# naver/panst3r

Measured on AMD Instinct MI355X. Metric: frames/sec (whole node), N-view 512px panoptic inference, higher is better.
Workload: dtype f16

## Files before the change

### include/panst3r_hip.h

```cpp
#ifndef PANST3R_HIP_H
#define PANST3R_HIP_H
#include <stdint.h>
#ifdef __cplusplus
extern "C" {
#endif

#define PST_ABI_VERSION 20

#define PST_BF16 0
#define PST_F32  1
#define PST_F16  2
#define PST_X3H  4

int pst_abi_version(void);
const char* pst_last_error(void);

typedef struct pst_gemm_params {
  const void* A;  int64_t lda;
  const void* W;  int64_t ldw;
  void* C;        int64_t ldc;
  int32_t M, N, K;
  const float* bias;
  const float* gamma;
  const float* res;  int64_t ldr;
// ... 6 lines not shown
  int32_t conv_c, conv_h, conv_w;
  const void* zeros;
  const int32_t* rope_pos; const float* rope_cs; int32_t rope_hd;
  int32_t rope_npos;
  int32_t res_bf16;
  int32_t kernel;
  int32_t batch;
  int64_t a_bs, w_bs, c_bs, bias_bs;
  int32_t dtype16;
  void* xcopy; int64_t ldxc;
  float* stats_out; int32_t stats_ld;
  const float* ln_stats; int32_t ln_groups; const float* ln_colsum; float ln_eps;
  int32_t x3_block;
} pst_gemm_params;

int pst_gemm(const pst_gemm_params* p, void* stream);
const char* pst_gemm_variant(const pst_gemm_params* p);
int pst_gemm_pair(const pst_gemm_params* a, const pst_gemm_params* b, void* stream);
const char* pst_gemm_pair_variant(const pst_gemm_params* a, const pst_gemm_params* b);
#define PST_TUNE_G256_PP 3
#define PST_TUNE_PAIR 4
#define PST_TUNE_DEEP_RING 8
#define PST_TUNE_PAIR_ATTN 7
#define PST_TUNE_ATTN_XCD 9
#define PST_TUNE_CUS 10
#define PST_TUNE_PAIR_DELAY 6
#define PST_TUNE_DEPHASE 11
#define PST_TUNE_PAIR_RES 5
int pst_tune(int knob, int value);

int pst_mask_head_supported(int Q, int P, int C);
int pst_mask_head(const void* E, int64_t lde, const void* F, int64_t f_view_stride, float* out, int64_t out_view_stride, int nviews, int Q, int P, int C,
                  int dtype16, void* stream);

typedef struct pst_attn_params {
  const void* Q;  int64_t q_bs, q_hs, q_rs;
  const void* K;  int64_t k_bs, k_hs, k_rs;
  const void* Vt; int64_t v_bs, v_hs, v_ds;
  void* O;        int64_t o_bs, o_hs, o_rs;
  const uint8_t* mask; int64_t m_bs, m_rs;
  int32_t B, H, Nq, Nk, hd;
  float scale;
  const void* zeros;
  int32_t nsplit;
  void* ws; int64_t ws_bytes;
  int32_t dtype16;
  int32_t prescaled;
} pst_attn_params;

int64_t pst_attn_workspace_bytes(int B, int H, int Nq, int hd, int nsplit);

int pst_attn_fwd(const pst_attn_params* p, void* stream);
const char* pst_attn_variant(const pst_attn_params* p);
int pst_attn_pair(const pst_attn_params* a, const pst_attn_params* b, void* stream);
const char* pst_attn_pair_variant(const pst_attn_params* a, const pst_attn_params* b);

int pst_layernorm(const void* x, int64_t ldx, int in_fp32, void* y, int64_t ldy, int out_fp32,
                  const float* gamma, const float* beta, int rows, int D, float eps,
                  int grp_in, int grp_out, int grp_off, void* stream);
int pst_layernorm_add(const void* x, int64_t ldx, int in_fp32, const float* add, int64_t ld_add, void* y, int64_t ldy,
                      int out_fp32, const float* gamma, const float* beta, int rows, int D, float eps,
                      int grp_in, int grp_out, int grp_off, void* stream);

int pst_token_embed(const int32_t* ids, int B, int L, const float* tok, int vocab, const float* pos, int npos, int D, float* out, int64_t ldo,
                    int32_t* status, void* stream);

int pst_rowstats(const void* x, int64_t ldx, int x_type, void* xcopy, int64_t ldxc, float* stats, int stats_ld, int rows, int D, int dtype16,
                 void* stream);

int pst_layernorm_add_batch(const void* x, int64_t ldx, int in_fp32, const float* add, int64_t ld_add, void* y, int64_t ldy,
                            int out_fp32, const float* gamma, const float* beta, int rows, int D, float eps,
                            int grp_in, int grp_out, int grp_off, int nbatch, int64_t x_bs, int64_t y_bs, int64_t w_bs,
                            void* stream);

int pst_split3(const float* x, int64_t ldx, void* out, int64_t ldo, int rows, int K, int dtype16, void* stream);

int pst_split_operand(const float* x, int64_t ldx, void* out, int64_t ldo, int rows, int K, int Kpad, int side, int dtype16, void* stream);
int pst_split2(const float* x, int64_t ldx, void* hi, void* lo, int64_t ldo, int rows, int K, int transpose, int dtype16, void* stream);
int pst_transpose_f32(const float* x, int64_t ldx, float* y, int64_t ldy, int rows, int cols, void* stream);
int pst_rope2d_split(const float* x, int64_t ld, const int32_t* pos, const float* cs, void* hi, void* lo, int64_t ldo, int rows, int nheads, int hd, int dtype16,
                     void* stream);
int pst_attn_x3(const pst_attn_params* p, const void* Q_lo, const void* K_lo, const void* Vt_lo, int out_type, int64_t out_block, void* stream);
const char* pst_attn_x3_variant(const pst_attn_params* p);

int pst_rope2d(void* x, int64_t ld, const int32_t* pos, const float* cs, int rows, int nheads, int hd, int dtype16,
               void* stream);

int pst_patchify(const float* img, void* out, int64_t ld, int nimg, int C, int H, int W, int p, int dtype16, void* stream);
int pst_dino_preprocess(const float* img, float* out, int nimg, int H, int W, int Ho, int Wo, void* stream);

int pst_image_prepare(const uint8_t* src, int Hs, int Ws, float* dst, int Hr, int Wr, int top, int left, int H, int W, void* stream);
int pst_patch_rows(const float* img, void* enc, int64_t ld_enc, void* dino, int64_t ld_dino, int nimg, int H, int W, int p_enc, int p_dino,
                   int dino_transposed, int dtype16, void* stream);

int pst_add_cast(const void* a, int64_t lda, int a_fp32, const void* b, int64_t ldb, int b_fp32, int b_mod,
                 void* y, int64_t ldy, int y_fp32, int rows, int D, void* stream);
int pst_l2norm_rows(const float* x, int64_t ldx, void* y, int64_t ldy, int rows, int D, float eps, int dtype16, void* stream);

int pst_mean4(const void* F, void* Fm, int nimg, int Hm, int Wm, int C, int dtype16, void* stream);
int pst_resize_bilinear(const void* F, void* Fd, int nimg, int Hs, int Ws, int Hd, int Wd, int C, int dtype16, void* stream);
int pst_attn_mask_from_logits(const float* logits, int64_t ldl, uint8_t* mask, int64_t ldm, int Q, int Nk,
                              void* stream);

#define PST_STATS_BLOCKS 128
int pst_loftup_guidance_gn(const float* img, const float* biases, const float* gamma, const float* beta, float eps,
                           float* scratch, float* stats, void* y, int64_t ldy, int nimg, int H, int W, int nf, int dtype16,
// ... 215 lines not shown
```

### panst3r_amd/csrc/attention.hip

```cpp
#include "common.h"
#include "../../include/panst3r_hip.h"

namespace pst {

constexpr int KT = 64;
constexpr float NEG = -1e30f;

template <int HD>
struct AttnCfg {
  static constexpr int KPITCH = (HD == 64) ? 128 : 256;
  static constexpr int KSLOTS = KPITCH / 16;
  static constexpr int KCHUNKS = HD / 8;
  static constexpr int K_BYTES = KT * KPITCH;
  static constexpr int V_BYTES = HD * 128;
  static constexpr int BUF = K_BYTES + V_BYTES;
  __device__ static __forceinline__ int kswz(int row) { return (HD == 64) ? ((row >> 1) & 7) : (row & 15); }
};

__device__ __forceinline__ float max_rows(float v) {
  const unsigned u = __float_as_uint(v);
  const auto a = __builtin_amdgcn_permlane16_swap(u, u, false, false);
  float m;
  asm("v_max_f32 %0, %1, %2" : "=v"(m) : "v"(a[0]), "v"(a[1]));
  const unsigned w = __float_as_uint(m);
  const auto b = __builtin_amdgcn_permlane32_swap(w, w, false, false);
  asm("v_max_f32 %0, %1, %2" : "=v"(m) : "v"(b[0]), "v"(b[1]));
  return m;
}

template <int HD, int QF, bool F16, bool PRE>
__device__ __forceinline__ void attn_body(const pst_attn_params& p, const int bidx, char* smem) {
  using C = AttnCfg<HD>;
  constexpr int NKK = HD / 32;
  constexpr int NHF = HD / 16;

  const int tid = threadIdx.x, lane = tid & 63;
  const int wave = __builtin_amdgcn_readfirstlane(tid >> 6);
  const int g = lane >> 4, l16 = lane & 15;

  const int qblocks = (p.Nq + 64 * QF - 1) / (64 * QF);
  const int nsplit = p.nsplit > 1 ? p.nsplit : 1;
  const int split = bidx % nsplit;
  const int bid = bidx / nsplit;
  const int qb = bid % qblocks, bh = bid / qblocks;
  const int h = bh % p.H, b = bh / p.H;

  const bf16_t* Qp = (const bf16_t*)p.Q + (int64_t)b * p.q_bs + (int64_t)h * p.q_hs;
  const bf16_t* Kp = (const bf16_t*)p.K + (int64_t)b * p.k_bs + (int64_t)h * p.k_hs;
  const bf16_t* Vp = (const bf16_t*)p.Vt + (int64_t)b * p.v_bs + (int64_t)h * p.v_hs;
  bf16_t* Op = (bf16_t*)p.O + (int64_t)b * p.o_bs + (int64_t)h * p.o_hs;
  const uint8_t* Mp = p.mask ? p.mask + (int64_t)b * p.m_bs : nullptr;

  const int q_wave0 = qb * (64 * QF) + wave * (16 * QF);
  bf16x8 qf[QF][NKK];
#pragma unroll
  for (int a = 0; a < QF; ++a) {
    const int q = min(q_wave0 + a * 16 + l16, p.Nq - 1);
#pragma unroll
    for (int kk = 0; kk < NKK; ++kk) qf[a][kk] = *(const bf16x8*)(Qp + (int64_t)q * p.q_rs + kk * 32 + g * 8);
  }

  constexpr int K_PER_THR = KT * C::KSLOTS / 256;
  constexpr int V_PER_THR = HD * 8 / 256;
  int k_key[K_PER_THR], k_chunk[K_PER_THR];
#pragma unroll
  for (int j = 0; j < K_PER_THR; ++j) {
    const int c = j * 256 + tid, row = c / C::KSLOTS, pos = c % C::KSLOTS;
    const int f = row >> 4, i = row & 15;
    k_key[j] = (f >> 1) * 32 + (i >> 2) * 8 + (f & 1) * 4 + (i & 3);
    k_chunk[j] = pos ^ C::kswz(row);
  }
  int v_row[V_PER_THR], v_chunk[V_PER_THR];
#pragma unroll
  for (int j = 0; j < V_PER_THR; ++j) {
    const int c = j * 256 + tid, row = c >> 3, pos = c & 7;
    v_row[j] = row;
    v_chunk[j] = pos ^ ((row >> 1) & 7);
  }

  uint32_t k_off[K_PER_THR], v_off[V_PER_THR];
#pragma unroll
  for (int j = 0; j < K_PER_THR; ++j) k_off[j] = (uint32_t)(k_key[j] * (int)p.k_rs + k_chunk[j] * 8) * 2u;
#pragma unroll
  for (int j = 0; j < V_PER_THR; ++j) v_off[j] = (uint32_t)(v_row[j] * (int)p.v_ds + v_chunk[j] * 8) * 2u;
  auto stage = [&](int kt, int buf) {
    const int k0 = kt * KT;
    char* kd = smem + buf * C::BUF + wave * 1024;
    char* vd = smem + buf * C::BUF + C::K_BYTES + wave * 1024;
    if (k0 + KT <= p.Nk) {
      const char* kbase = (const char*)Kp + (int64_t)k0 * p.k_rs * 2;
      const char* vbase = (const char*)Vp + (int64_t)k0 * 2;
#pragma unroll
      for (int j = 0; j < K_PER_THR; ++j)
        if (C::KSLOTS == C::KCHUNKS || k_chunk[j] < C::KCHUNKS) glds16(kbase + k_off[j], kd + j * 4096);
#pragma unroll
      for (int j = 0; j < V_PER_THR; ++j) glds16(vbase + v_off[j], vd + j * 4096);
      return;
    }
#pragma unroll
    for (int j = 0; j < K_PER_THR; ++j) {
      if (C::KSLOTS == C::KCHUNKS || k_chunk[j] < C::KCHUNKS) {
        const int key = min(k0 + k_key[j], p.Nk - 1);
        glds16(Kp + (int64_t)key * p.k_rs + k_chunk[j] * 8, kd + j * 4096);
      }
    }
#pragma unroll
    for (int j = 0; j < V_PER_THR; ++j) {
      const int kcol = k0 + v_chunk[j] * 8;
      const bf16_t* s = (kcol < p.Nk) ? Vp + (int64_t)v_row[j] * p.v_ds + kcol : (const bf16_t*)p.zeros;
      glds16(s, vd + j * 4096);
    }
  };

  f32x4 o[NHF][QF];
#pragma unroll
  for (int hf = 0; hf < NHF; ++hf)
#pragma unroll
    for (int a = 0; a < QF; ++a) o[hf][a] = f32x4{0.f, 0.f, 0.f, 0.f};
  f32x4 negm[QF];
  float m_run[QF], lsum[QF];
  float sum_lim[QF];
#pragma unroll
  for (int a = 0; a < QF; ++a) { m_run[a] = NEG; negm[a] = f32x4{0.f, 0.f, 0.f, 0.f}; lsum[a] = 0.f; sum_lim[a] = -1.0f; }
  bf16x8 ones;
  {
    union { bf16x8 v; uint32_t u[4]; } t;
    t.u[0] = t.u[1] = t.u[2] = t.u[3] = F16 ? 0x3c003c00u : 0x3f803f80u;
    ones = t.v;
    asm volatile("" : "+v"(ones));
  }

  const float c_exp = PRE ? 1.0f : p.scale * 1.4426950408889634f;
  const float lazy_thr = 8.0f / c_exp;
  const int tiles_all = (p.Nk + KT - 1) / KT;
  const int tps = (tiles_all + nsplit - 1) / nsplit;
  const int kt_begin = split * tps;
  const int ntiles = min(tiles_all, kt_begin + tps);
  if (kt_begin < ntiles) stage(kt_begin, 0);
  for (int kt = kt_begin; kt < ntiles; ++kt) {
#ifndef PST_ABL_NOSTAGE
    wait_vm0();
    __syncthreads();
    if (kt + 1 < ntiles) stage(kt + 1, (kt + 1 - kt_begin) & 1);
    const char* kb_ = smem + ((kt - kt_begin) & 1) * C::BUF;
#else
    if (kt == kt_begin) { wait_vm0(); __syncthreads(); }
    const char* kb_ = smem;
#endif
    const char* vb_ = kb_ + C::K_BYTES;
    const int k0 = kt * KT;
    if (q_wave0 >= p.Nq) continue;

    const bool tail = (k0 + KT > p.Nk);
    bool fast = !Mp && !tail && kt > kt_begin;
    bool trip[QF];
#pragma unroll
    for (int a = 0; a < QF; ++a) trip[a] = false;
    bf16x8 pb[QF][2];
    f32x4 tsum[QF];
    for (;;) {
      asm volatile("" ::: "memory");
      f32x4 s[4][QF];
#pragma unroll
      for (int f = 0; f < 4; ++f) {
#pragma unroll
        for (int a = 0; a < QF; ++a) s[f][a] = negm[a];
        const int row = f * 16 + l16;
#pragma unroll
        for (int kk = 0; kk < NKK; ++kk) {
          const int kc = kk * 4 + g;
          const bf16x8 kf = *(const bf16x8*)(kb_ + row * C::KPITCH + ((kc ^ C::kswz(row)) << 4));
#pragma unroll
          for (int a = 0; a < QF; ++a) s[f][a] = H16<F16>::mfma(kf, qf[a][kk], s[f][a]);
        }
      }

      if (!fast) {
        int k0c = k0;
        asm volatile("" : "+s"(k0c));
        float mx[QF];
#pragma unroll
        for (int a = 0; a < QF; ++a) {
          const int q = q_wave0 + a * 16 + l16;
          if (Mp || tail) {
            const uint8_t* mrow = Mp ? Mp + (int64_t)min(q, p.Nq - 1) * p.m_rs : nullptr;
#pragma unroll
            for (int f = 0; f < 4; ++f) {
              const int key = k0c + (f >> 1) * 32 + g * 8 + (f & 1) * 4;
              uint32_t mb = 0;
              if (mrow && key < p.Nk) mb = *(const uint32_t*)(mrow + key);
#pragma unroll
              for (int r = 0; r < 4; ++r)
                if (key + r >= p.Nk || ((mb >> (8 * r)) & 0xff)) s[f][a][r] = NEG;
            }
          }
          auto max3 = [](float x, float y, float z) { return fmaxf(fmaxf(x, y), z); };
          float m0 = max3(s[0][a][0], s[0][a][1], s[0][a][2]), m1 = max3(s[2][a][0], s[2][a][1], s[2][a][2]);
          m0 = max3(m0, s[0][a][3], s[1][a][0]); m1 = max3(m1, s[2][a][3], s[3][a][0]);
          m0 = max3(m0, s[1][a][1], s[1][a][2]); m1 = max3(m1, s[3][a][1], s[3][a][2]);
          mx[a] = fmaxf(max3(m0, m1, s[1][a][3]), s[3][a][3]);
        }
// ... 28 lines not shown
      }

#pragma unroll
      for (int a = 0; a < QF; ++a) {
        float pv[4][4];
#pragma unroll
        for (int f = 0; f < 4; ++f)
#pragma unroll
          for (int r = 0; r < 4; ++r) {
#ifndef PST_ABL_NOEXP
            pv[f][r] = __builtin_amdgcn_exp2f(PRE ? s[f][a][r] : s[f][a][r] * c_exp);
#else
            pv[f][r] = s[f][a][r];
#endif
          }
#pragma unroll
        for (int kb = 0; kb < 2; ++kb) {
          union { bf16x8 v; uint32_t u[4]; } pk;
          pk.u[0] = H16<F16>::pack(pv[2 * kb][0], pv[2 * kb][1]);
          pk.u[1] = H16<F16>::pack(pv[2 * kb][2], pv[2 * kb][3]);
          pk.u[2] = H16<F16>::pack(pv[2 * kb + 1][0], pv[2 * kb + 1][1]);
          pk.u[3] = H16<F16>::pack(pv[2 * kb + 1][2], pv[2 * kb + 1][3]);
          pb[a][kb] = pk.v;
        }
        tsum[a] = H16<F16>::mfma(ones, pb[a][0], f32x4{0.f, 0.f, 0.f, 0.f});
        tsum[a] = H16<F16>::mfma(ones, pb[a][1], tsum[a]);
      }
      if (!fast) break;
      uint64_t tripped = 0;
#pragma unroll
      for (int a = 0; a < QF; ++a) {
        trip[a] = !(tsum[a][0] <= sum_lim[a]);
        tripped |= __builtin_amdgcn_ballot_w64(trip[a]);
      }
      if (tripped == 0) break;
      fast = false;
    }

#pragma unroll
    for (int a = 0; a < QF; ++a) lsum[a] += tsum[a][0];
#pragma unroll
    for (int hf = 0; hf < NHF; ++hf) {
      const int row = hf * 16 + l16;
#pragma unroll
      for (int kb = 0; kb < 2; ++kb) {
        const int vc = kb * 4 + g;
        const bf16x8 vf = *(const bf16x8*)(vb_ + row * 128 + ((vc ^ ((row >> 1) & 7)) << 4));
#pragma unroll
        for (int a = 0; a < QF; ++a) o[hf][a] = H16<F16>::mfma(vf, pb[a][kb], o[hf][a]);
      }
    }
  }

  if (nsplit > 1) {
    float* ws_o = (float*)p.ws;
    const int64_t rows = (int64_t)p.B * p.H * p.Nq;
    float* ws_ml = ws_o + (int64_t)nsplit * rows * HD;
#pragma unroll
    for (int a = 0; a < QF; ++a) {
      const float l = lsum[a];
      const int q = q_wave0 + a * 16 + l16;
      if (q < p.Nq) {
        const int64_t row = ((int64_t)b * p.H + h) * p.Nq + q;
        float* dst = ws_o + ((int64_t)split * rows + row) * HD + 4 * g;
#pragma unroll
        for (int hf = 0; hf < NHF; ++hf) *(float4*)(dst + hf * 16) = make_float4(o[hf][a][0], o[hf][a][1], o[hf][a][2], o[hf][a][3]);
        if (g == 0) *(float2*)(ws_ml + ((int64_t)split * rows + row) * 2) = make_float2(m_run[a], l);
      }
    }
    return;
  }

#pragma unroll
  for (int a = 0; a < QF; ++a) {
    const float l = lsum[a];
    const float inv = l > 0.f ? 1.0f / l : 0.f;
    const int q = q_wave0 + a * 16 + l16;
    if (q < p.Nq) {
      bf16_t* dst = Op + (int64_t)q * p.o_rs + 4 * g;
#pragma unroll
      for (int hf = 0; hf < NHF; ++hf)
        *(uint2*)(dst + hf * 16) = make_uint2(H16<F16>::pack(o[hf][a][0] * inv, o[hf][a][1] * inv),
                                              H16<F16>::pack(o[hf][a][2] * inv, o[hf][a][3] * inv));
    }
  }
}

template <int HD, int QF, bool F16, bool PRE>
__global__ __launch_bounds__(256) void attn_kernel(const pst_attn_params p, const int xcd) {
  extern __shared__ __attribute__((aligned(16))) char smem[];
  attn_body<HD, QF, F16, PRE>(p, xcd ? xcd_remap((int)blockIdx.x, (int)gridDim.x) : (int)blockIdx.x, smem);
}

struct attn2_args {
  pst_attn_params p[2];
  int nblk0;
};
template <int HD, int QF, bool F16, bool PRE>
__global__ __launch_bounds__(256) void attn2_kernel(const attn2_args a, const int xcd) {
  extern __shared__ __attribute__((aligned(16))) char smem[];
  const int blk = xcd ? xcd_remap((int)blockIdx.x, (int)gridDim.x) : (int)blockIdx.x;
  const int which = blk >= a.nblk0 ? 1 : 0;
  attn_body<HD, QF, F16, PRE>(a.p[which], which ? blk - a.nblk0 : blk, smem);
}

__global__ void attn_combine_kernel(const pst_attn_params p, int hd) {
  const int64_t rows = (int64_t)p.B * p.H * p.Nq;
  const int per_row = hd / 4;
  const int64_t total = rows * per_row;
  const float c_exp = p.prescaled ? 1.0f : p.scale * 1.4426950408889634f;
  const float* ws_o = (const float*)p.ws;
  const float* ws_ml = ws_o + (int64_t)p.nsplit * rows * hd;
  for (int64_t i = blockIdx.x * (int64_t)blockDim.x + threadIdx.x; i < total; i += (int64_t)gridDim.x * blockDim.x) {
    const int64_t row = i / per_row;
    const int d = (int)(i - row * per_row) * 4;
    float m = NEG;
    for (int s = 0; s < p.nsplit; ++s) m = fmaxf(m, ws_ml[((int64_t)s * rows + row) * 2]);
    float l = 0.f, acc[4] = {0.f, 0.f, 0.f, 0.f};
    for (int s = 0; s < p.nsplit; ++s) {
      const float2 ml = *(const float2*)(ws_ml + ((int64_t)s * rows + row) * 2);
      const float wgt = __builtin_amdgcn_exp2f((ml.x - m) * c_exp);
      const float4 v = *(const float4*)(ws_o + ((int64_t)s * rows + row) * hd + d);
      l += ml.y * wgt;
      acc[0] += v.x * wgt; acc[1] += v.y * wgt; acc[2] += v.z * wgt; acc[3] += v.w * wgt;
    }
    const float inv = l > 0.f ? 1.0f / l : 0.f;
    const int q = (int)(row % p.Nq);
    const int bh = (int)(row / p.Nq), h = bh % p.H, b = bh / p.H;
    bf16_t* dst = (bf16_t*)p.O + (int64_t)b * p.o_bs + (int64_t)h * p.o_hs + (int64_t)q * p.o_rs + d;
    *(uint2*)dst = make_uint2(pack2(acc[0] * inv, acc[1] * inv, p.dtype16), pack2(acc[2] * inv, acc[3] * inv, p.dtype16));
  }
}

static int g_attn_xcd = 1;
int attn_xcd_order(int set) { const int prev = g_attn_xcd; if (set == 0 || set == 1) g_attn_xcd = set; return prev; }

template <int HD, int QF, bool F16, bool PRE>
static int launch_attn4(const pst_attn_params& p, hipStream_t s) {
  const int qblocks = (p.Nq + 64 * QF - 1) / (64 * QF);
  const int nsplit = p.nsplit > 1 ? p.nsplit : 1;
  const long grid = (long)qblocks * p.H * p.B * nsplit;
  hipLaunchKernelGGL((attn_kernel<HD, QF, F16, PRE>), dim3((unsigned)grid), dim3(256), 2 * AttnCfg<HD>::BUF, s, p, attn_xcd_order(-1));
  if (nsplit > 1) {
    const int64_t total = (int64_t)p.B * p.H * p.Nq * (HD / 4);
    int64_t g = (total + 255) / 256;
    if (g > 4096) g = 4096;
    hipLaunchKernelGGL(attn_combine_kernel, dim3((unsigned)g), dim3(256), 0, s, p, HD);
  }
  return check_launch("attn_fwd");
}

template <int HD, int QF, bool F16>
static int launch_attn(const pst_attn_params& p, hipStream_t s) {
  return p.prescaled ? launch_attn4<HD, QF, F16, true>(p, s) : launch_attn4<HD, QF, F16, false>(p, s);
}

template <int HD, int QF, bool F16, bool PRE>
static int launch_attn2_t(const pst_attn_params& pa, const pst_attn_params& pb, hipStream_t s) {
  attn2_args a;
  a.p[0] = pa; a.p[1] = pb;
  const long ga = (long)((pa.Nq + 64 * QF - 1) / (64 * QF)) * pa.H * pa.B, gb = (long)((pb.Nq + 64 * QF - 1) / (64 * QF)) * pb.H * pb.B;
  a.nblk0 = (int)ga;
  hipLaunchKernelGGL((attn2_kernel<HD, QF, F16, PRE>), dim3((unsigned)(ga + gb)), dim3(256), 2 * AttnCfg<HD>::BUF, s, a, attn_xcd_order(-1));
  return check_launch("attn_fwd (pair)");
}

int attn_f32_validate(const pst_attn_params& p);
int launch_attn_f32(const pst_attn_params& p, hipStream_t s);

}

static int attn_validate(const pst_attn_params* pp) {
  using namespace pst;
  if (!pp) { set_error("attn: null params"); return PST_EINVAL; }
  const pst_attn_params& p = *pp;
  if (p.dtype16 == DT_F32) {
    if (p.prescaled != 0 && p.prescaled != 1) { set_error("attn: prescaled must be 0 or 1"); return PST_EINVAL; }
    if (!p.prescaled && !(p.scale > 0.f)) { set_error("attn: scale must be positive"); return PST_EINVAL; }
    if (p.B <= 0 || p.H <= 0 || p.Nq <= 0 || p.Nk <= 0 || !p.Q || !p.K || !p.Vt || !p.O) { set_error("attn: bad shape / null operand"); return PST_EINVAL; }
    return attn_f32_validate(p);
  }
  if (p.dtype16 != DT_BF16 && p.dtype16 != DT_F16) { set_error("attn: dtype16 must be PST_BF16, PST_F16 or PST_F32"); return PST_EINVAL; }
  if (p.prescaled != 0 && p.prescaled != 1) { set_error("attn: prescaled must be 0 or 1"); return PST_EINVAL; }
  if (!p.prescaled && !(p.scale > 0.f)) { set_error("attn: scale must be positive"); return PST_EINVAL; }
  if (p.hd != 64 && p.hd != 96) { set_error("attn: head dim %d unsupported (64 or 96)", p.hd); return PST_EINVAL; }
  if (p.B <= 0 || p.H <= 0 || p.Nq <= 0 || p.Nk <= 0) { set_error("attn: bad shape"); return PST_EINVAL; }
  if (!p.Q || !p.K || !p.Vt || !p.O || !p.zeros) { set_error("attn: null operand"); return PST_EINVAL; }
  if ((p.q_rs | p.q_hs | p.q_bs | p.k_rs | p.k_hs | p.k_bs | p.v_ds | p.v_hs | p.v_bs) % 8) {
    set_error("attn: Q/K/Vt strides must be multiples of 8 elements (16-byte rows)"); return PST_EINVAL;
  }
  if ((p.o_rs | p.o_hs | p.o_bs) % 4) { set_error("attn: O strides must be multiples of 4"); return PST_EINVAL; }
  if (((uintptr_t)p.Q | (uintptr_t)p.K | (uintptr_t)p.Vt) & 15 || ((uintptr_t)p.O & 7)) {
    set_error("attn: operands must be 16-byte aligned"); return PST_EINVAL;
  }
  if (p.k_rs < 0) { set_error("attn: k_rs must not be negative"); return PST_EINVAL; }
  if (p.v_ds < 0) { set_error("attn: v_ds must not be negative"); return PST_EINVAL; }
  if (p.k_rs * 64 * 2 >= (1ll << 31) || p.v_ds * (int64_t)p.hd * 2 >= (1ll << 31)) { set_error("attn: K row / V^T row stride too large"); return PST_EINVAL; }
  if (p.mask && ((p.m_rs | p.m_bs) % 4 || ((uintptr_t)p.mask & 3))) { set_error("attn: mask rows must be 4-byte aligned"); return PST_EINVAL; }
  if (p.nsplit > 1) {
    const int64_t need = (int64_t)p.nsplit * p.B * p.H * p.Nq * (p.hd + 2) * 4;
    if (!p.ws || p.ws_bytes < need || ((uintptr_t)p.ws & 15)) { set_error("attn: split-K needs a 16-byte aligned workspace of %lld bytes", (long long)need); return PST_EINVAL; }
    if (p.nsplit > 64) { set_error("attn: nsplit <= 64"); return PST_EINVAL; }
  }
  return PST_OK;
}

static bool attn_big(const pst_attn_params& p) { return (long)((p.Nq + 127) / 128) * p.H * p.B * (p.nsplit > 1 ? p.nsplit : 1) >= 256; }

extern "C" int pst_attn_fwd(const pst_attn_params* pp, void* stream) {
  using namespace pst;
  if (int rc = attn_validate(pp)) return rc;
  const pst_attn_params& p = *pp;
  hipStream_t s = (hipStream_t)stream;
  if (p.dtype16 == DT_F32) return launch_attn_f32(p, s);
  const bool big = attn_big(p), h = p.dtype16 == DT_F16;
  if (p.hd == 64) {
    if (big) return h ? launch_attn<64, 2, true>(p, s) : launch_attn<64, 2, false>(p, s);
    return h ? launch_attn<64, 1, true>(p, s) : launch_attn<64, 1, false>(p, s);
  }
  if (big) return h ? launch_attn<96, 2, true>(p, s) : launch_attn<96, 2, false>(p, s);
  return h ? launch_attn<96, 1, true>(p, s) : launch_attn<96, 1, false>(p, s);
}

static int g_attn_pair = 1;
namespace pst { int attn_pair_enable(int set) { const int prev = g_attn_pair; if (set == 0 || set == 1) g_attn_pair = set; return prev; } }

static bool attn_pair_fusable(const pst_attn_params& a, const pst_attn_params& b) {
  if (!g_attn_pair) return false;
  if (a.dtype16 == pst::DT_F32 || a.dtype16 != b.dtype16 || a.hd != b.hd || a.prescaled != b.prescaled || a.nsplit > 1 || b.nsplit > 1) return false;
  if (!a.prescaled && a.scale != b.scale) return false;
  return attn_big(a) && attn_big(b);
}

extern "C" int pst_attn_pair(const pst_attn_params* pa, const pst_attn_params* pb, void* stream) {
  using namespace pst;
  if (int rc = attn_validate(pa)) return rc;
  if (int rc = attn_validate(pb)) return rc;
  if (!attn_pair_fusable(*pa, *pb)) {
    if (int rc = pst_attn_fwd(pa, stream)) return rc;
    return pst_attn_fwd(pb, stream);
  }
  hipStream_t s = (hipStream_t)stream;
  const bool h = pa->dtype16 == DT_F16, pre = pa->prescaled != 0;
#define PST_A2(HD) (h ? (pre ? launch_attn2_t<HD, 2, true, true>(*pa, *pb, s) : launch_attn2_t<HD, 2, true, false>(*pa, *pb, s)) \
                      : (pre ? launch_attn2_t<HD, 2, false, true>(*pa, *pb, s) : launch_attn2_t<HD, 2, false, false>(*pa, *pb, s)))
  return pa->hd == 64 ? PST_A2(64) : PST_A2(96);
#undef PST_A2
}

extern "C" const char* pst_attn_pair_variant(const pst_attn_params* pa, const pst_attn_params* pb) {
  if (attn_validate(pa) || attn_validate(pb)) return nullptr;
  if (!attn_pair_fusable(*pa, *pb)) return "";
  return pa->hd == 64 ? "attn2_kernel<64,2>" : "attn2_kernel<96,2>";
}

extern "C" const char* pst_attn_variant(const pst_attn_params* pp) {
  if (attn_validate(pp)) return nullptr;
  if (pp->dtype16 == pst::DT_F32) return pp->hd == 64 ? "attn_f32_kernel<64>" : "attn_f32_kernel<96>";
  const bool big = attn_big(*pp);
  if (pp->hd == 64) return big ? "attn_kernel<64,2>" : "attn_kernel<64,1>";
  return big ? "attn_kernel<96,2>" : "attn_kernel<96,1>";
}

extern "C" int64_t pst_attn_workspace_bytes(int B, int H, int Nq, int hd, int nsplit) {
  return nsplit > 1 ? (int64_t)nsplit * B * H * Nq * (hd + 2) * 4 : 0;
}
```

### panst3r_amd/hip.py

```python
import ctypes as C
import os
import torch

_HERE = os.path.dirname(os.path.abspath(__file__))
LIB_PATH = os.environ.get('PST_LIB') or os.path.join(_HERE, 'lib', 'libpanst3r_hip.so')
ABI_VERSION = 20
STATS_BLOCKS = 128
_lib = None

i32, i64, f32, vp = C.c_int32, C.c_int64, C.c_float, C.c_void_p


class GemmParams(C.Structure):
    _fields_ = [('A', vp), ('lda', i64), ('W', vp), ('ldw', i64), ('C', vp), ('ldc', i64),
                ('M', i32), ('N', i32), ('K', i32),
                ('bias', vp), ('gamma', vp), ('res', vp), ('ldr', i64), ('res_mod', i32),
                ('act', i32), ('out_fp32', i32), ('trans_out', i32),
                ('grp_in', i32), ('grp_out', i32), ('grp_off', i32),
                ('ps_p', i32), ('ps_c', i32), ('ps_h', i32), ('ps_w', i32),
                ('conv_c', i32), ('conv_h', i32), ('conv_w', i32), ('zeros', vp), ('rope_pos', vp), ('rope_cs', vp), ('rope_hd', i32), ('rope_npos', i32), ('res_bf16', i32), ('kernel', i32),
                ('batch', i32), ('a_bs', i64), ('w_bs', i64), ('c_bs', i64), ('bias_bs', i64), ('dtype16', i32),
                ('xcopy', vp), ('ldxc', i64), ('stats_out', vp), ('stats_ld', i32), ('ln_stats', vp), ('ln_groups', i32), ('ln_colsum', vp), ('ln_eps', f32), ('x3_block', i32)]


class AttnParams(C.Structure):
    _fields_ = [('Q', vp), ('q_bs', i64), ('q_hs', i64), ('q_rs', i64),
                ('K', vp), ('k_bs', i64), ('k_hs', i64), ('k_rs', i64),
                ('Vt', vp), ('v_bs', i64), ('v_hs', i64), ('v_ds', i64),
                ('O', vp), ('o_bs', i64), ('o_hs', i64), ('o_rs', i64),
                ('mask', vp), ('m_bs', i64), ('m_rs', i64),
                ('B', i32), ('H', i32), ('Nq', i32), ('Nk', i32), ('hd', i32),
                ('scale', f32), ('zeros', vp), ('nsplit', i32), ('ws', vp), ('ws_bytes', i64), ('dtype16', i32), ('prescaled', i32)]


class CloudView(C.Structure):
    _fields_ = [('conf', vp), ('pts3d', vp), ('pts3d_local', vp), ('img', vp), ('pan', vp), ('offset', i64), ('npix', i32), ('first_wg', i32), ('c2w', f32 * 12)]


_CODES = {'i': C.c_int, 'l': C.c_int64, 'u': C.c_uint64, 'f': C.c_float, 'd': C.c_double, 'p': vp, 's': C.c_char_p,
          'G': C.POINTER(GemmParams), 'A': C.POINTER(AttnParams)}
SIGNATURES = {
    'pst_abi_version': 'i:', 'pst_last_error': 's:', 'pst_gemm': 'i:Gp', 'pst_gemm_variant': 's:G', 'pst_gemm_pair': 'i:GGp', 'pst_gemm_pair_variant': 's:GG',
    'pst_tune': 'i:ii', 'pst_mask_head_supported': 'i:iii', 'pst_mask_head': 'i:plplpliiiiip', 'pst_attn_workspace_bytes': 'l:iiiii', 'pst_attn_fwd': 'i:Ap',
    'pst_attn_variant': 's:A', 'pst_attn_pair': 'i:AAp', 'pst_attn_pair_variant': 's:AA', 'pst_layernorm': 'i:pliplippiifiiip',
    'pst_layernorm_add': 'i:pliplplippiifiiip', 'pst_token_embed': 'i:piipipiiplpp', 'pst_rowstats': 'i:pliplpiiiip',
    'pst_layernorm_add_batch': 'i:pliplplippiifiiiilllp', 'pst_split3': 'i:plpliiip', 'pst_split_operand': 'i:plpliiiiip', 'pst_split2': 'i:plppliiiip',
    'pst_transpose_f32': 'i:plpliip', 'pst_rope2d_split': 'i:plppppliiiip', 'pst_attn_x3': 'i:Apppilp', 'pst_attn_x3_variant': 's:A',
    'pst_rope2d': 'i:plppiiiip', 'pst_patchify': 'i:ppliiiiiip', 'pst_dino_preprocess': 'i:ppiiiiip', 'pst_image_prepare': 'i:piipiiiiiip',
    'pst_patch_rows': 'i:pplpliiiiiiip', 'pst_add_cast': 'i:plipliipliiip', 'pst_l2norm_rows': 'i:plpliifip', 'pst_mean4': 'i:ppiiiiip',
    'pst_resize_bilinear': 'i:ppiiiiiiip', 'pst_attn_mask_from_logits': 'i:plpliip', 'pst_loftup_guidance_gn': 'i:ppppfpppliiiiipp',
    'pst_loftup_minmax': 'i:ppiiip', 'pst_minmax_merge': 'i:pppip', 'pst_groupnorm_stats': 'i:plipiiiip', 'pst_groupnorm_apply': 'i:plippppliiiifiip',
    'pst_loftup_lr_pe': 'i:ppliiiiip', 'pst_pp_scores': 'i:piiffpppp', 'pst_pp_scores_softmax': 'i:piifpppp', 'pst_pp_sigmoid': 'i:pppiip',
    'pst_pp_argmax': 'i:pppiiiiifppppp', 'pst_pp_argmax_logits': 'i:pppiiiiifppppp', 'pst_pp_select': 'i:pppidppp', 'pst_pp_finalize': 'i:pppiffppp',
    'pst_qubo_upsample': 'i:ppiiiiip', 'pst_qubo_workspace_floats': 'l:il', 'pst_qubo_overlap': 'i:pilppp', 'pst_qubo_argmax': 'i:ppilppp',
    'pst_pointmap_activate': 'i:pppplip', 'pst_focal_weiszfeld': 'i:pppiiiip', 'pst_rigid_moments': 'i:ppppiifp', 'pst_retrieval_select': 'i:plppiiiplpp',
    'pst_retrieval_assign': 'i:plplpiiiiippppip', 'pst_retrieval_aggregate': 'i:plplpppiippp', 'pst_retrieval_scores': 'i:ppppppiiiiffpp',
    'pst_cloud_count': 'i:piifpp', 'pst_cloud_scan': 'i:pipp', 'pst_cloud_compact': 'i:piifppiffppppppp', 'pst_cloud_segment_median': 'i:ppplpiippppppp',
    'pst_qubo_anneal_max_n': 'i:', 'pst_qubo_anneal': 'i:piiifffuppppp',
    'pst_voxel_insert': 'i:plfplpppip', 'pst_voxel_count': 'i:pplpp', 'pst_voxel_rank': 'i:pplpppp', 'pst_voxel_accumulate': 'i:ppplfpppipppplppip',
    'pst_voxel_vote': 'i:pplpp', 'pst_voxel_emit': 'i:pppplfdppppiffppppppp',
    'pst_render_max_radius': 'i:', 'pst_render_splat': 'i:plpiiifiipip', 'pst_render_resolve': 'i:pllppppppppp',
    'pst_consist_depth': 'i:ppiilfipp', 'pst_consist_count': 'i:pppiilfippppp',
    'pst_tsdf_insert': 'i:pliplpppp', 'pst_tsdf_nodes': 'i:pliplplppppp', 'pst_tsdf_integrate': 'i:plfipppipppp', 'pst_tsdf_cells': 'i:plplpppipppp',
    'pst_tsdf_vertices': 'i:plplpppippppldppppppp', 'pst_tsdf_face_count': 'i:plplpppippppp', 'pst_tsdf_face_emit': 'i:plplppppppppppp',
    'pst_mesh_lane_pixels': 'i:', 'pst_mesh_raster': 'i:plplpiiiffppplip', 'pst_mesh_resolve': 'i:piiiplplpfpppppp', 'pst_mesh_area_count': 'i:pilpiipp',
    'pst_mesh_area_apply': 'i:pilpiipipp',
    'pst_pq_count': 'i:pplpipipiiipip', 'pst_pq_match': 'i:piiipppppppp',
    'pst_vcc_cells': 'i:ppplfpp', 'pst_vcc_build': 'i:pplpplppp', 'pst_vcc_link': 'i:pplpplippp', 'pst_vcc_flatten': 'i:ppplppppppip', 'pst_vcc_count': 'i:plpp',
    'pst_vcc_rank': 'i:pplpppppppppppppp', 'pst_vcc_votes': 'i:pppplppliipplpp', 'pst_vcc_apply': 'i:pppplippiffpppp',
    'pst_surface_rows': 'i:pllpp', 'pst_surface_count': 'i:ppiipfpp', 'pst_surface_emit': 'i:ppiipfpppppp', 'pst_surface_link': 'i:pllpppp',
    'pst_surface_components': 'i:pllppppp', 'pst_surface_keep_count': 'i:pplipp', 'pst_surface_keep_emit': 'i:ppppplippppp',
    'pst_mesh_sample_count': 'i:plplfipppp', 'pst_mesh_sample_emit': 'i:plplpllppppppp',
    'pst_nn_insert': 'i:plfplpppp', 'pst_nn_scatter': 'i:plpppppp', 'pst_nn_query': 'i:plplffplpppipppp',
    'pst_icp_chunk': 'i:', 'pst_icp_step': 'i:plffffffffffffplffplpppipppppp',
    'pst_meshdist_count': 'i:plplfpppp', 'pst_meshdist_insert': 'i:plplfplplpppp', 'pst_meshdist_scatter': 'i:ppllpppppp',
    'pst_meshdist_query': 'i:plplplffplppplippppp',
    'pst_plane_icp_step': 'i:plfffffffffffffffplplffplppplipppppp',
    'pst_depth_median': 'i:ppiiifffpppppp', 'pst_depth_moments': 'i:ppiipifffppp', 'pst_depth_errors': 'i:ppiipifffpiddddppp',
}
EXPORTS = list(SIGNATURES)


def lib():
    global _lib
    if _lib is not None:
        return _lib
    if not os.path.exists(LIB_PATH):
        raise RuntimeError('libpanst3r_hip.so not found at %s -- run `python -m panst3r_amd.build` (hipcc, gfx950). '
                           'The HIP path has no fallback.' % LIB_PATH)
    L = C.CDLL(LIB_PATH)
    for name, sig in SIGNATURES.items():
        ret, args = sig.split(':')
        fn = getattr(L, name)
        fn.restype, fn.argtypes = _CODES[ret], [_CODES[c] for c in args]
    if L.pst_abi_version() != ABI_VERSION:
        raise RuntimeError('libpanst3r_hip.so ABI %d != expected %d; rebuild' % (L.pst_abi_version(), ABI_VERSION))
    _lib = L
# ... 444 lines not shown
def gemm_pair(first, second):
    (a1, w1, o1, k1), (a2, w2, o2, k2) = first, second
    t32 = lambda a, o, k: k.get('trans_out') and o.dtype == torch.float32 and a.dtype in H16
    if t32(a1, o1, k1) or t32(a2, o2, k2):
        gemm(a1, w1, o1, **k1)
        gemm(a2, w2, o2, **k2)
        return o1, o2
    if _x3_wanted(a1, w1) or _x3_wanted(a2, w2):
        fin = []
        if _x3_wanted(a1, w1):
            a1, w1, o1x, k1, f = _x3_prepare(a1, w1, o1, k1)
            fin.append(f)
        else:
            o1x = o1
        if _x3_wanted(a2, w2):
            a2, w2, o2x, k2, f = _x3_prepare(a2, w2, o2, k2)
            fin.append(f)
        else:
            o2x = o2
        gemm_pair((a1, w1, o1x, k1), (a2, w2, o2x, k2))
        for f in fin:
            if f is not None:
                f()
        return o1, o2
    p1, f1, t1 = _gemm_params(a1, w1, o1, **k1)
    p2, f2, t2 = _gemm_params(a2, w2, o2, **k2)
    name = _variant('pst_gemm_pair_variant', '', p1, p2) if TIMER is not None else None
    if name == '':
        gemm(a1, w1, o1, **k1)
        gemm(a2, w2, o2, **k2)
        return o1, o2
    _timed(name, f1 + f2, t1 + t2, _call, 'pst_gemm_pair', p1, p2)
    if MAXABS is not None and TIMER is None:
        _note_gemm(o1, k1, t1)
        _note_gemm(o2, k2, t2)
    return o1, o2


def mask_head_supported(Q, P, C):
    return bool(lib().pst_mask_head_supported(Q, P, C))


def mask_head(embed, feats, out):
    _dev(embed, *H16); _dev(feats, *H16); _dev(out, torch.float32)
    n, C = feats.shape[0], feats.shape[-1]
    P = feats.numel() // (n * C)
    Q = embed.shape[0]
    assert feats.is_contiguous() and out.is_contiguous() and out.numel() == n * Q * P and embed.shape[1] == C and embed.stride(1) == 1
    _timed('mask_head_kernel', 2.0 * n * Q * P * C, ('bytes', float(n * (C * P * 2 + Q * P * 4))), _call,
           'pst_mask_head', _ptr(embed), embed.stride(0), _ptr(feats), P * C, _ptr(out), Q * P, n, Q, P, C, _same16(embed, feats))
    return out


def auto_nsplit(B, H, Nq, Nk):
    blocks = ((Nq + 63) // 64) * H * B
    if blocks >= 256 or Nk < 1024:
        return 1
    blocks128 = ((Nq + 127) // 128) * H * B
    if Nk >= 5376:
        ns = min(512 // blocks128, Nk // 768, 12) if Nk <= 12288 else min(768 // blocks128, Nk // 1024, 12)
        if blocks128 * ns >= 256:
            return ns
    return max(1, min(512 // blocks, Nk // 512, 32))


LOG2E = 1.4426950408889634


def attn_workspace_floats(B, H, Nq, Nk, hd, nsplit=None):
    ns = auto_nsplit(B, H, Nq, Nk) if nsplit is None else nsplit
    return ns * B * H * Nq * (hd + 2) if ns > 1 else 0


def _attn_struct(fmt, q, k, vt, out, B, H, Nq, Nk, hd, q_strides, k_strides, v_strides, o_strides, scale, mask, mask_strides, ns, ws, prescaled):
    p = AttnParams()
    p.dtype16 = fmt
    p.Q, (p.q_bs, p.q_hs, p.q_rs) = q, q_strides
    p.K, (p.k_bs, p.k_hs, p.k_rs) = k, k_strides
    p.Vt, (p.v_bs, p.v_hs, p.v_ds) = vt, v_strides
    p.O, (p.o_bs, p.o_hs, p.o_rs) = _ptr(out), o_strides
    if mask is not None:
        _dev(mask, torch.uint8)
        p.mask, (p.m_bs, p.m_rs) = _ptr(mask), mask_strides
    p.B, p.H, p.Nq, p.Nk, p.hd = B, H, Nq, Nk, hd
    p.scale = float(hd ** -0.5 if scale is None else scale)
    p.prescaled = 1 if prescaled else 0
    p.zeros = _ptr(zeros_page(out.device))
    if ns > 1:
        n = attn_workspace_floats(B, H, Nq, Nk, hd, ns)
        if ws is None:
            ws = torch.empty(n, dtype=torch.float32, device=out.device)
        assert ws.dtype == torch.float32 and ws.numel() >= n
        p.nsplit, p.ws, p.ws_bytes = ns, _ptr(ws), ws.numel() * 4
    return p, ws


def _attn_params(q, k, vt, out, B, H, Nq, Nk, hd, q_strides, k_strides, v_strides, o_strides, scale=None, mask=None,
                 mask_strides=(0, 0), nsplit=None, ws=None, prescaled=False):
    _dev(q, *FMT); _dev(k, *FMT); _dev(vt, *FMT); _dev(out, *FMT)
    ns = auto_nsplit(B, H, Nq, Nk) if nsplit is None else nsplit
    if q.dtype == torch.float32 and nsplit is None:
        ns = 1
    p, ws = _attn_struct(_fmt(q, k, vt, out), _ptr(q), _ptr(k), _ptr(vt), out, B, H, Nq, Nk, hd, q_strides, k_strides, v_strides, o_strides,
                         scale, mask, mask_strides, ns, ws, prescaled)
    return p, ws, 4.0 * B * H * Nq * Nk * hd, (B, H, Nq, Nk, hd)


def attention(q, k, vt, out, B, H, Nq, Nk, hd, q_strides, k_strides, v_strides, o_strides, scale=None, mask=None,
              mask_strides=(0, 0), nsplit=None, ws=None, prescaled=False):
    if (isinstance(q, Planes) or q.dtype == torch.float32) and X3:
        return _attention_x3(q, k, vt, out, B, H, Nq, Nk, hd, q_strides, k_strides, v_strides, o_strides, scale, mask, mask_strides, nsplit, ws, prescaled)
    p, ws, flops, tag = _attn_params(q, k, vt, out, B, H, Nq, Nk, hd, q_strides, k_strides, v_strides, o_strides, scale, mask, mask_strides, nsplit, ws, prescaled)
    _timed(lambda: _variant('pst_attn_variant', 'attn?', p), flops, tag, _call, 'pst_attn_fwd', p)
    if TIMER is None:
        note_maxabs(out, 'attention hd=%d out' % hd)
    return out


def _span(B, H, N, strides, width):
    bs, hs, rs = strides
    offs = [b * bs + h * hs + r * rs for b in (0, B - 1) for h in (0, H - 1) for r in (0, N - 1)]
    return min(offs), max(offs) + width


def _attention_x3(q, k, vt, out, B, H, Nq, Nk, hd, q_strides, k_strides, v_strides, o_strides, scale, mask, mask_strides, nsplit, ws, prescaled):
    _dev(out, torch.float32, X3_FMT)
    out_type, out_block = (1, 0) if out.dtype == torch.float32 else (X3H, out.shape[-1] // 3)
    dev = out.device
    spans = []
    for t, (lo_, hi_) in ((q, _span(B, H, Nq, q_strides, hd)), (k, _span(B, H, Nk, k_strides, hd)),
                          (vt, _span(B, H, hd, v_strides, (Nk + 7) // 8 * 8))):
        if isinstance(t, Planes):
            continue
        _dev(t, torch.float32)
        spans.append([t.data_ptr() + 4 * lo_, t.data_ptr() + 4 * ((hi_ + 3) // 4 * 4)])
    merged = []
    for a0, a1 in sorted(spans):
        if merged and a0 <= merged[-1][1]:
            merged[-1][1] = max(merged[-1][1], a1)
        else:
            merged.append([a0, a1])
    planes = []
    for a0, a1 in merged:
        n = (a1 - a0) // 4
        assert a0 % 16 == 0 and n % 4 == 0, 'attention operands must be 16-byte aligned with strides that are multiples of 8'
        hi = torch.empty(n, dtype=X3_FMT, device=dev)
        lo = torch.empty(n, dtype=X3_FMT, device=dev)
        _call('pst_split2', a0, n, _ptr(hi), _ptr(lo), n, 1, n, 0, _TC[X3_FMT])
        planes.append((a0, a1, hi, lo))

    def plane_ptrs(t):
        if isinstance(t, Planes):
            return t.hi.data_ptr(), t.lo.data_ptr()
# ... 1117 lines not shown
```

Baseline: 330.6.

## Split attention keys across wave groups inside one workgroup, merging via LDS

Adds a key-group attention variant where a workgroup runs 2 or 4 groups of four waves. Each group processes a disjoint share of the key tiles for the same 64-query block, and the partial outputs are merged through shared memory in-kernel. For mid-sized grids this replaces the global-workspace split-K plus separate merge kernel, aiming to fill the GPU without an extra launch and workspace traffic. It costs larger workgroups and more LDS per block, and the Python heuristic now disables split-K for hd=64 at 128+ blocks so those shapes take the key-group path.

Result: slower. 325.1 (-1.6%).

```diff
diff --git a/include/panst3r_hip.h b/include/panst3r_hip.h
--- a/include/panst3r_hip.h
+++ b/include/panst3r_hip.h
@@ -82,6 +82,7 @@
 
 int pst_attn_fwd(const pst_attn_params* p, void* stream);
 const char* pst_attn_variant(const pst_attn_params* p);
+int pst_attn_key_groups(const pst_attn_params* p);
 int pst_attn_pair(const pst_attn_params* a, const pst_attn_params* b, void* stream);
 const char* pst_attn_pair_variant(const pst_attn_params* a, const pst_attn_params* b);
 
diff --git a/panst3r_amd/csrc/attention.hip b/panst3r_amd/csrc/attention.hip
--- a/panst3r_amd/csrc/attention.hip
+++ b/panst3r_amd/csrc/attention.hip
@@ -28,18 +28,39 @@
   return m;
 }
 
-template <int HD, int QF, bool F16, bool PRE>
-__device__ __forceinline__ void attn_body(const pst_attn_params& p, const int bidx, char* smem) {
+template <class ML, class VAL>
+__device__ __forceinline__ void attn_merge(const int n, const float c_exp, ML ml, VAL val, float (&out)[4]) {
+  float m = NEG;
+  for (int s = 0; s < n; ++s) m = fmaxf(m, ml(s).x);
+  float l = 0.f, acc[4] = {0.f, 0.f, 0.f, 0.f};
+  for (int s = 0; s < n; ++s) {
+    const float2 x = ml(s);
+    const float wgt = __builtin_amdgcn_exp2f((x.x - m) * c_exp);
+    const float4 v = val(s);
+    l = __builtin_fmaf(x.y, wgt, l);
+    acc[0] = __builtin_fmaf(v.x, wgt, acc[0]); acc[1] = __builtin_fmaf(v.y, wgt, acc[1]);
+    acc[2] = __builtin_fmaf(v.z, wgt, acc[2]); acc[3] = __builtin_fmaf(v.w, wgt, acc[3]);
+  }
+  const float inv = l > 0.f ? 1.0f / l : 0.f;
+#pragma unroll
+  for (int r = 0; r < 4; ++r) out[r] = acc[r] * inv;
+}
+
+template <int HD, int QF, bool F16, bool PRE, int KG = 1>
+__device__ __forceinline__ void attn_body(const pst_attn_params& p, const int bidx, char* smem_block) {
   using C = AttnCfg<HD>;
   constexpr int NKK = HD / 32;
   constexpr int NHF = HD / 16;
-
-  const int tid = threadIdx.x, lane = tid & 63;
+  static_assert(KG == 1 || QF == 1, "key groups: 64-query blocks only");
+
+  const int tid = KG > 1 ? (int)(threadIdx.x & 255) : (int)threadIdx.x, lane = tid & 63;
   const int wave = __builtin_amdgcn_readfirstlane(tid >> 6);
+  const int kgrp = KG > 1 ? __builtin_amdgcn_readfirstlane((int)threadIdx.x >> 8) : 0;
+  char* const smem = smem_block + kgrp * (2 * C::BUF);
   const int g = lane >> 4, l16 = lane & 15;
 
   const int qblocks = (p.Nq + 64 * QF - 1) / (64 * QF);
-  const int nsplit = p.nsplit > 1 ? p.nsplit : 1;
+  const int nsplit = (KG == 1 && p.nsplit > 1) ? p.nsplit : 1;
   const int split = bidx % nsplit;
   const int bid = bidx / nsplit;
   const int qb = bid % qblocks, bh = bid / qblocks;
@@ -133,11 +154,13 @@
   const float c_exp = PRE ? 1.0f : p.scale * 1.4426950408889634f;
   const float lazy_thr = 8.0f / c_exp;
   const int tiles_all = (p.Nk + KT - 1) / KT;
-  const int tps = (tiles_all + nsplit - 1) / nsplit;
-  const int kt_begin = split * tps;
+  const int parts = KG > 1 ? KG : nsplit, part = KG > 1 ? kgrp : split;
+  const int tps = (tiles_all + parts - 1) / parts;
+  const int kt_begin = part * tps;
   const int ntiles = min(tiles_all, kt_begin + tps);
+  const int kt_end = KG > 1 ? kt_begin + tps : ntiles;
   if (kt_begin < ntiles) stage(kt_begin, 0);
-  for (int kt = kt_begin; kt < ntiles; ++kt) {
+  for (int kt = kt_begin; kt < kt_end; ++kt) {
 #ifndef PST_ABL_NOSTAGE
     wait_vm0();
     __syncthreads();
@@ -147,6 +170,7 @@
     if (kt == kt_begin) { wait_vm0(); __syncthreads(); }
     const char* kb_ = smem;
 #endif
+    if (KG > 1 && kt >= ntiles) continue;
     const char* vb_ = kb_ + C::K_BYTES;
     const int k0 = kt * KT;
     if (q_wave0 >= p.Nq) continue;
@@ -281,6 +305,40 @@
     }
   }
 
+  if constexpr (KG > 1) {
+    static_assert((NHF + 1) * 4096 <= 2 * C::BUF, "key groups: the partial results must fit the group's ring");
+    __syncthreads();
+    const bool live = q_wave0 < p.Nq;
+    if (kgrp > 0 && live) {
+      float4* dst = (float4*)(smem + wave * ((NHF + 1) * 1024)) + lane;
+#pragma unroll
+      for (int hf = 0; hf < NHF; ++hf) dst[hf * 64] = make_float4(o[hf][0][0], o[hf][0][1], o[hf][0][2], o[hf][0][3]);
+      dst[NHF * 64] = make_float4(m_run[0], lsum[0], 0.f, 0.f);
+    }
+    __syncthreads();
+    if (kgrp > 0 || !live) return;
+    const int q = q_wave0 + l16;
+    float2 ml[KG];
+    ml[0] = make_float2(m_run[0], lsum[0]);
+#pragma unroll
+    for (int s = 1; s < KG; ++s) {
+      const float4 t = ((const float4*)(smem_block + s * (2 * C::BUF) + wave * ((NHF + 1) * 1024)))[NHF * 64 + lane];
+      ml[s] = make_float2(t.x, t.y);
+    }
+    bf16_t* dst = Op + (int64_t)q * p.o_rs + 4 * g;
+#pragma unroll
+    for (int hf = 0; hf < NHF; ++hf) {
+      float4 v[KG];
+      v[0] = make_float4(o[hf][0][0], o[hf][0][1], o[hf][0][2], o[hf][0][3]);
+#pragma unroll
+      for (int s = 1; s < KG; ++s) v[s] = ((const float4*)(smem_block + s * (2 * C::BUF) + wave * ((NHF + 1) * 1024)))[hf * 64 + lane];
+      float r[4];
+      attn_merge(KG, c_exp, [&](int s) { return ml[s]; }, [&](int s) { return v[s]; }, r);
+      if (q < p.Nq) *(uint2*)(dst + hf * 16) = make_uint2(H16<F16>::pack(r[0], r[1]), H16<F16>::pack(r[2], r[3]));
+    }
+    return;
+  }
+
   if (nsplit > 1) {
     float* ws_o = (float*)p.ws;
     const int64_t rows = (int64_t)p.B * p.H * p.Nq;
@@ -315,10 +373,10 @@
   }
 }
 
-template <int HD, int QF, bool F16, bool PRE>
-__global__ __launch_bounds__(256) void attn_kernel(const pst_attn_params p, const int xcd) {
+template <int HD, int QF, bool F16, bool PRE, int KG = 1>
+__global__ __launch_bounds__(256 * KG) void attn_kernel(const pst_attn_params p, const int xcd) {
   extern __shared__ __attribute__((aligned(16))) char smem[];
-  attn_body<HD, QF, F16, PRE>(p, xcd ? xcd_remap((int)blockIdx.x, (int)gridDim.x) : (int)blockIdx.x, smem);
+  attn_body<HD, QF, F16, PRE, KG>(p, xcd ? xcd_remap((int)blockIdx.x, (int)gridDim.x) : (int)blockIdx.x, smem);
 }
 
 struct attn2_args {
@@ -343,21 +401,13 @@
   for (int64_t i = blockIdx.x * (int64_t)blockDim.x + threadIdx.x; i < total; i += (int64_t)gridDim.x * blockDim.x) {
     const int64_t row = i / per_row;
     const int d = (int)(i - row * per_row) * 4;
-    float m = NEG;
-    for (int s = 0; s < p.nsplit; ++s) m = fmaxf(m, ws_ml[((int64_t)s * rows + row) * 2]);
-    float l = 0.f, acc[4] = {0.f, 0.f, 0.f, 0.f};
-    for (int s = 0; s < p.nsplit; ++s) {
-      const float2 ml = *(const float2*)(ws_ml + ((int64_t)s * rows + row) * 2);
-      const float wgt = __builtin_amdgcn_exp2f((ml.x - m) * c_exp);
-      const float4 v = *(const float4*)(ws_o + ((int64_t)s * rows + row) * hd + d);
-      l += ml.y * wgt;
-      acc[0] += v.x * wgt; acc[1] += v.y * wgt; acc[2] += v.z * wgt; acc[3] += v.w * wgt;
-    }
-    const float inv = l > 0.f ? 1.0f / l : 0.f;
+    float r[4];
+    attn_merge(p.nsplit, c_exp, [&](int s) { return *(const float2*)(ws_ml + ((int64_t)s * rows + row) * 2); },
+               [&](int s) { return *(const float4*)(ws_o + ((int64_t)s * rows + row) * hd + d); }, r);
     const int q = (int)(row % p.Nq);
     const int bh = (int)(row / p.Nq), h = bh % p.H, b = bh / p.H;
     bf16_t* dst = (bf16_t*)p.O + (int64_t)b * p.o_bs + (int64_t)h * p.o_hs + (int64_t)q * p.o_rs + d;
-    *(uint2*)dst = make_uint2(pack2(acc[0] * inv, acc[1] * inv, p.dtype16), pack2(acc[2] * inv, acc[3] * inv, p.dtype16));
+    *(uint2*)dst = make_uint2(pack2(r[0], r[1], p.dtype16), pack2(r[2], r[3], p.dtype16));
   }
 }
 
@@ -384,6 +434,21 @@
   return p.prescaled ? launch_attn4<HD, QF, F16, true>(p, s) : launch_attn4<HD, QF, F16, false>(p, s);
 }
 
+template <int HD, bool F16, bool PRE, int KG>
+static int launch_attn_kg4(const pst_attn_params& p, hipStream_t s) {
+  static unsigned long long seen = 0;
+  once_per_device(seen, [] { (void)hipFuncSetAttribute((const void*)attn_kernel<HD, 1, F16, PRE, KG>, hipFuncAttributeMaxDynamicSharedMemorySize, KG * 2 * AttnCfg<HD>::BUF); });
+  const long grid = (long)((p.Nq + 63) / 64) * p.H * p.B;
+  hipLaunchKernelGGL((attn_kernel<HD, 1, F16, PRE, KG>), dim3((unsigned)grid), dim3(256 * KG), KG * 2 * AttnCfg<HD>::BUF, s, p, attn_xcd_order(-1));
+  return check_launch("attn_fwd (key groups)");
+}
+
+template <int HD, int KG>
+static int launch_attn_kg(const pst_attn_params& p, hipStream_t s) {
+  if (p.dtype16 == DT_F16) return p.prescaled ? launch_attn_kg4<HD, true, true, KG>(p, s) : launch_attn_kg4<HD, true, false, KG>(p, s);
+  return p.prescaled ? launch_attn_kg4<HD, false, true, KG>(p, s) : launch_attn_kg4<HD, false, false, KG>(p, s);
+}
+
 template <int HD, int QF, bool F16, bool PRE>
 static int launch_attn2_t(const pst_attn_params& pa, const pst_attn_params& pb, hipStream_t s) {
   attn2_args a;
@@ -431,10 +496,22 @@
     if (!p.ws || p.ws_bytes < need || ((uintptr_t)p.ws & 15)) { set_error("attn: split-K needs a 16-byte aligned workspace of %lld bytes", (long long)need); return PST_EINVAL; }
     if (p.nsplit > 64) { set_error("attn: nsplit <= 64"); return PST_EINVAL; }
   }
+  if (p.nsplit < 0 && p.nsplit != -2 && !(p.nsplit == -4 && p.hd == 64)) {
+    set_error("attn: nsplit %d: the key groups of a workgroup are 2, or 4 at head dim 64", p.nsplit); return PST_EINVAL;
+  }
   return PST_OK;
 }
 
 static bool attn_big(const pst_attn_params& p) { return (long)((p.Nq + 127) / 128) * p.H * p.B * (p.nsplit > 1 ? p.nsplit : 1) >= 256; }
+
+static int attn_key_groups(const pst_attn_params& p) {
+  if (p.dtype16 == pst::DT_F32 || p.nsplit > 1) return 1;
+  if (p.nsplit < 0) return -p.nsplit;
+  if ((long)((p.Nq + 63) / 64) * p.H * p.B >= 256) return 1;
+  const int tiles = (p.Nk + pst::KT - 1) / pst::KT;
+  if (p.hd == 64 && tiles >= 8) return 4;
+  return tiles >= 4 ? 2 : 1;
+}
 
 extern "C" int pst_attn_fwd(const pst_attn_params* pp, void* stream) {
   using namespace pst;
@@ -442,6 +519,11 @@
   const pst_attn_params& p = *pp;
   hipStream_t s = (hipStream_t)stream;
   if (p.dtype16 == DT_F32) return launch_attn_f32(p, s);
+  const int kg = attn_key_groups(p);
+  if (kg > 1) {
+    if (p.hd == 64) return kg == 4 ? launch_attn_kg<64, 4>(p, s) : launch_attn_kg<64, 2>(p, s);
+    return launch_attn_kg<96, 2>(p, s);
+  }
   const bool big = attn_big(p), h = p.dtype16 == DT_F16;
   if (p.hd == 64) {
     if (big) return h ? launch_attn<64, 2, true>(p, s) : launch_attn<64, 2, false>(p, s);
@@ -455,7 +537,7 @@
 namespace pst { int attn_pair_enable(int set) { const int prev = g_attn_pair; if (set == 0 || set == 1) g_attn_pair = set; return prev; } }
 
 static bool attn_pair_fusable(const pst_attn_params& a, const pst_attn_params& b) {
-  if (!g_attn_pair) return false;
+  if (!g_attn_pair || a.nsplit < 0 || b.nsplit < 0) return false;
   if (a.dtype16 == pst::DT_F32 || a.dtype16 != b.dtype16 || a.hd != b.hd || a.prescaled != b.prescaled || a.nsplit > 1 || b.nsplit > 1) return false;
   if (!a.prescaled && a.scale != b.scale) return false;
   return attn_big(a) && attn_big(b);
@@ -486,11 +568,16 @@
 extern "C" const char* pst_attn_variant(const pst_attn_params* pp) {
   if (attn_validate(pp)) return nullptr;
   if (pp->dtype16 == pst::DT_F32) return pp->hd == 64 ? "attn_f32_kernel<64>" : "attn_f32_kernel<96>";
-  const bool big = attn_big(*pp);
+  const bool big = pp->nsplit >= 0 && attn_big(*pp);
   if (pp->hd == 64) return big ? "attn_kernel<64,2>" : "attn_kernel<64,1>";
   return big ? "attn_kernel<96,2>" : "attn_kernel<96,1>";
 }
 
+extern "C" int pst_attn_key_groups(const pst_attn_params* pp) {
+  if (attn_validate(pp)) return -1;
+  return attn_key_groups(*pp);
+}
+
 extern "C" int64_t pst_attn_workspace_bytes(int B, int H, int Nq, int hd, int nsplit) {
   return nsplit > 1 ? (int64_t)nsplit * B * H * Nq * (hd + 2) * 4 : 0;
 }
diff --git a/panst3r_amd/hip.py b/panst3r_amd/hip.py
--- a/panst3r_amd/hip.py
+++ b/panst3r_amd/hip.py
@@ -42,7 +42,7 @@
 SIGNATURES = {
     'pst_abi_version': 'i:', 'pst_last_error': 's:', 'pst_gemm': 'i:Gp', 'pst_gemm_variant': 's:G', 'pst_gemm_pair': 'i:GGp', 'pst_gemm_pair_variant': 's:GG',
     'pst_tune': 'i:ii', 'pst_mask_head_supported': 'i:iii', 'pst_mask_head': 'i:plplpliiiiip', 'pst_attn_workspace_bytes': 'l:iiiii', 'pst_attn_fwd': 'i:Ap',
-    'pst_attn_variant': 's:A', 'pst_attn_pair': 'i:AAp', 'pst_attn_pair_variant': 's:AA', 'pst_layernorm': 'i:pliplippiifiiip',
+    'pst_attn_variant': 's:A', 'pst_attn_key_groups': 'i:A', 'pst_attn_pair': 'i:AAp', 'pst_attn_pair_variant': 's:AA', 'pst_layernorm': 'i:pliplippiifiiip',
     'pst_layernorm_add': 'i:pliplplippiifiiip', 'pst_token_embed': 'i:piipipiiplpp', 'pst_rowstats': 'i:pliplpiiiip',
     'pst_layernorm_add_batch': 'i:pliplplippiifiiiilllp', 'pst_split3': 'i:plpliiip', 'pst_split_operand': 'i:plpliiiiip', 'pst_split2': 'i:plppliiiip',
     'pst_transpose_f32': 'i:plpliip', 'pst_rope2d_split': 'i:plppppliiiip', 'pst_attn_x3': 'i:Apppilp', 'pst_attn_x3_variant': 's:A',
@@ -593,9 +593,11 @@
     return out
 
 
-def auto_nsplit(B, H, Nq, Nk):
+def auto_nsplit(B, H, Nq, Nk, hd=None):
     blocks = ((Nq + 63) // 64) * H * B
     if blocks >= 256 or Nk < 1024:
+        return 1
+    if hd == 64 and blocks >= 128 and Nk <= 5376:
         return 1
     blocks128 = ((Nq + 127) // 128) * H * B
     if Nk >= 5376:
@@ -609,7 +611,7 @@
 
 
 def attn_workspace_floats(B, H, Nq, Nk, hd, nsplit=None):
-    ns = auto_nsplit(B, H, Nq, Nk) if nsplit is None else nsplit
+    ns = auto_nsplit(B, H, Nq, Nk, hd) if nsplit is None else nsplit
     return ns * B * H * Nq * (hd + 2) if ns > 1 else 0
 
 
@@ -633,13 +635,15 @@
             ws = torch.empty(n, dtype=torch.float32, device=out.device)
         assert ws.dtype == torch.float32 and ws.numel() >= n
         p.nsplit, p.ws, p.ws_bytes = ns, _ptr(ws), ws.numel() * 4
+    elif ns < 0:
+        p.nsplit = ns
     return p, ws
 
 
 def _attn_params(q, k, vt, out, B, H, Nq, Nk, hd, q_strides, k_strides, v_strides, o_strides, scale=None, mask=None,
                  mask_strides=(0, 0), nsplit=None, ws=None, prescaled=False):
     _dev(q, *FMT); _dev(k, *FMT); _dev(vt, *FMT); _dev(out, *FMT)
-    ns = auto_nsplit(B, H, Nq, Nk) if nsplit is None else nsplit
+    ns = auto_nsplit(B, H, Nq, Nk, hd) if nsplit is None else nsplit
     if q.dtype == torch.float32 and nsplit is None:
         ns = 1
     p, ws = _attn_struct(_fmt(q, k, vt, out), _ptr(q), _ptr(k), _ptr(vt), out, B, H, Nq, Nk, hd, q_strides, k_strides, v_strides, o_strides,
```
